# MadNLP/MadNLP.jl

Measured on AMD Instinct MI355X. Metric: IP iterations/sec + ms per factorize!/solve!, condensed KKT n≈1e4, higher is better.
Workload: dtype f64; 1 GPU; BASELINE config C3: case1354pegase-shaped sparse-condensed KKT, one instance; N=11192, m=16646, nnz(K)=68688; step = compress_J+compress_H+build_kkt+factorize (n_f=1) + inertia fetch + 2 solve_linear_system per instance; algorithm=BUNCHKAUFMAN (device: static-pivot LDL^T), outer_block=0, batch_per_gpu=1, batch_api=n/a (one instance), parallelism=1 GPU(s) x 1 independent instance(s)

## Files before the change

### madnlp.jl_amd/_lib.py

```python
from __future__ import annotations

import ctypes as C
import os
import subprocess

_HERE = os.path.dirname(os.path.abspath(__file__))
CSRC = os.path.join(_HERE, "csrc")
LIBDIR = os.path.join(_HERE, "lib")
LIBPATH = os.path.join(LIBDIR, "libmadnlp_hip.so")
_LIB_OVERRIDE = os.environ.get("MNK_LIBPATH")
SOURCES = ["gemm_f64.hip", "dag.hip", "dag_plan.hip", "dag_batch.hip", "factor.hip", "factor_plan.hip", "solve.hip", "ls.hip", "ls_alt.hip", "sparse_kkt.hip", "dense_kkt.hip", "bk.hip", "schur.hip", "ipm_vec.hip", "opf_eval.hip", "qr.hip", "lu.hip", "evd.hip", "qn.hip", "tape_eval.hip", "nlp_scale.hip"]
HEADERS = ["common.h", "ls.h", "dag_plan.h", "factor_plan.h", "kkt_vec.h", "gemm_tile.h", "leaf64.h", "ipm_handle.h", os.path.join("..", "..", "include", "madnlp_hip.h")]

MNK_HOST, MNK_DEVICE = 0, 1
MNK_BUNCHKAUFMAN, MNK_LU, MNK_QR, MNK_CHOLESKY, MNK_LDL, MNK_EVD = 1, 2, 3, 4, 5, 6
MNK_SC_JT, MNK_SC_HESS, MNK_SC_AUG, MNK_SC_DIAGBUF = 0, 1, 2, 3
MNK_QN_BFGS, MNK_QN_DAMPED_BFGS = 1, 2


def _stale() -> bool:
    if not os.path.exists(LIBPATH):
        return True
    t = os.path.getmtime(LIBPATH)
    deps = [os.path.join(CSRC, s) for s in SOURCES + HEADERS]
    return any(os.path.exists(d) and os.path.getmtime(d) > t for d in deps)


FILE_FLAGS = {"gemm_f64.hip": ["-mllvm", "-amdgpu-mfma-vgpr-form"], "dag.hip": ["-mllvm", "-amdgpu-mfma-vgpr-form"],
              "bk.hip": ["-mllvm", "-amdgpu-mfma-vgpr-form"]}


def build(force: bool = False, verbose: bool = False) -> str:
    if not force and not _stale():
        return LIBPATH
    from concurrent.futures import ThreadPoolExecutor
    hipcc = os.environ.get("HIPCC", "/opt/rocm/bin/hipcc")
    os.makedirs(LIBDIR, exist_ok=True)
    objdir = os.path.join(LIBDIR, "obj")
    os.makedirs(objdir, exist_ok=True)
    base = [hipcc, "--offload-arch=gfx950", "-O3", "-std=c++17", "-fPIC"]

    def compile_one(src):
        obj = os.path.join(objdir, src.replace(".hip", ".o"))
        cmd = base + FILE_FLAGS.get(src, []) + ["-c", os.path.join(CSRC, src), "-o", obj]
        if verbose:
# ... 240 lines not shown
```

### madnlp.jl_amd/csrc/ls.h

```cpp
#pragma once
#include <algorithm>
#include <functional>
#include <memory>
#include <string>
#include <vector>

#include "common.h"
#include "dag_plan.h"
#include "factor_plan.h"

struct mnk_sc {
    mnk_ctx* ctx = nullptr;
    int64_t n = 0, m = 0, nnzj = 0, nnzh = 0;
    int64_t nnz_jt = 0, nnz_hess = 0, nnz_aug = 0, len_jptr = 0;
    std::vector<int32_t> jt_colptr, jt_rowval, h_colptr, h_rowval, aug_colptr, aug_rowval;
    std::vector<int32_t> tile_env;
    mnk::DevBuf<int32_t> d_tile_env;
    std::vector<int32_t> tile_envh;
    mnk::DevBuf<int32_t> d_tile_envh;
    std::vector<int64_t> jt_map, h_map;
    std::vector<int32_t> d_dst, d_src, hp_dst, hp_src, j_dst, j_c, j_k, j_l;
    mnk::DevBuf<int32_t> jt_seg_ptr, jt_seg_src, h_seg_ptr, h_seg_src;
    mnk::DevBuf<int32_t> aug_hptr, aug_hsrc;
    mnk::DevBuf<int32_t> aug_dsrc;
// ... 167 lines not shown
    double bk_growth_tol = 64.0, bk_growth_tol_qd = 1e8;
    double last_growth = 0.0;
    int64_t last_sign_changes = 0;
    int count = 0;
    mnk::DevBuf<unsigned long long> amax_dev;
    bool wanted(const mnk_ls* ls) const;
    unsigned long long* growth_word(const mnk_ls* ls) const;
    bool guard_fetched(const mnk_ls* ls) const;
    bool may_take_over(const mnk_ls* ls) const;
    void note_growth(double am, double dm, int64_t sign_changes) { last_growth = am > 0.0 ? dm / am : (dm > 0.0 ? HUGE_VAL : 0.0); last_sign_changes = sign_changes; }
    bool grew() const { return !(last_growth <= (last_sign_changes <= 1 ? bk_growth_tol_qd : bk_growth_tol)); }
    int run(mnk_ls* ls);
    int permute(mnk_ls* ls, double* x, double* tmp, bool forward);
    int dsolve(mnk_ls* ls, double* y);
    int inertia(mnk_ls* ls, unsigned long long* out_dev);
    int read_pivots(mnk_ls* ls, int32_t* perm_host, double* doff_host);
    bool multi_last() const { return ran_multi; }
    int mw_fallbacks() const { return n_mw_fallbacks; }
   private:
    int factor(mnk_ls* ls, bool multi);
    mnk::DevBuf<int> perm, ptype;
    mnk::DevBuf<double> doff, dcoup, work;
    mnk::DevBuf<char> state;
    mnk::DevBuf<double> wv, tmp; mnk::DevBuf<unsigned long long> msg; mnk::DevBuf<int> aux;
    bool ran_multi = false, mw_blocked = false;
    int n_mw_fallbacks = 0;
};

struct SolveState {
    int persistent_solve = 1;
    int solve512 = 0;
    int linv_mfma = 1;
    long ps_spin_limit = 6000000;
    int debug_ps_missing = -1;
    mnk::DevBuf<double> linv512, linv512t, linv512tmp;
    mnk::DevBuf<unsigned long long> trace;
    int create();
    void destroy();
    int* abort_word() const { return abort; }
    bool abort_raised() const { return abort && *abort != 0; }
    bool take_abort();
    int poll_buffer() const { return pub_next; }
    bool reset_due(int b) { const bool due = !pub_clean[b]; pub_clean[b] = true; return due; }
    void dirtied(int b) { pub_clean[b] = false; }
    void solve_queued(bool other_cleared) { pub_clean[pub_next] = false; pub_clean[pub_next ^ 1] = other_cleared; pub_next ^= 1; }
   private:
    int* abort = nullptr;
    int pub_next = 0;
    bool pub_clean[2] = {false, false};
};

struct mnk_ls {
    mnk_ctx* ctx = nullptr;
    int64_t N = 0, Np = 0, ld = 0, ldw = 0, nbo = 512;
    bool nbo_auto = true;
    int algo = MNK_LDL;
    double pivot_tol = 0.0;
    int lookahead = 1;
    int share = 1;
    int small_tiles = 400;
    int64_t single_rows = 2560;
    mnk::DevBuf<int> tile_ctr;
    mnk::DevBuf<double> fact, wbuf[2], linv, dblk, inv16, linv256, linv256t, dvec, dinv, xwork;
    SpareFill spare;
    int epoch = 0;
    mnk::DevBuf<int> flag_p;
// ... 124 lines not shown
```

### madnlp.jl_amd/csrc/ls.hip

```cpp
#include <cstdarg>
#include <cstdlib>
#include <atomic>
#include <map>
#include <mutex>

#include <cfloat>
#include "ls.h"

namespace mnk {

static thread_local std::string g_err;
void set_error(const char* fmt, ...) {
    char buf[1024];
    va_list ap;
    va_start(ap, fmt);
    vsnprintf(buf, sizeof(buf), fmt, ap);
    va_end(ap);
    g_err = buf;
}

__global__ __launch_bounds__(256) void fill_lower_kernel(double* __restrict__ F, int64_t ld, int64_t N, int64_t Np) {
    const int64_t col = blockIdx.x;
    const int64_t first = (col / PAD) * PAD;
    const int64_t r = first + ((int64_t)blockIdx.y * 256 + threadIdx.x) * 2;
// ... 669 lines not shown
    if (!strcmp(key, "accept_only_pd")) { ls->accept_only_pd = value != 0; return 0; }
    if (!strcmp(key, "probe")) { ls->probe.on = value != 0; return 0; }
    if (!strcmp(key, "early_reject")) { ls->early_reject = value != 0; return 0; }
    if (!strcmp(key, "dag_debug")) {
        ls->dag_debug = value != 0.0;
        if (ls->dag_debug && !ls->dag_dbg.p) {
            if (ls->dag_dbg.alloc(8 * 128 + 16 * 1024)) return -2;
            MNK_HIP(hipMemset(ls->dag_dbg.p, 0, (8 * 128 + 16 * 1024) * sizeof(int)));
        }
        return 0;
    }
    if (!strcmp(key, "bk_max_wgs")) {
        MNK_REQUIRE(value >= 0.0 && value <= 256.0, "bk_max_wgs must be in 0..256");
        ls->bk.bk_max_wgs = (int)value;
        return 0;
    }
    if (!strcmp(key, "bk_spin_limit")) {
        MNK_REQUIRE(value >= 1024.0, "bk_spin_limit must be at least 1024");
        ls->bk.bk_spin_limit = (long)value;
        return 0;
    }
    if (!strcmp(key, "debug_bk_missing")) { ls->bk.debug_bk_missing = (int)value; return 0; }
    if (!strcmp(key, "bk_growth_tol")) {
        MNK_REQUIRE(value > 1.0, "bk_growth_tol must be > 1");
        ls->bk.bk_growth_tol = value;
        return 0;
    }
    if (!strcmp(key, "bk_growth_tol_qd")) {
        MNK_REQUIRE(value > 1.0, "bk_growth_tol_qd must be > 1");
        ls->bk.bk_growth_tol_qd = value;
        return 0;
    }
    if (!strcmp(key, "persistent_solve")) { ls->solves.persistent_solve = value != 0.0; return 0; }
    if (!strcmp(key, "ps_spin_limit")) {
        MNK_REQUIRE(value >= 1024.0, "ps_spin_limit must be at least 1024");
        ls->solves.ps_spin_limit = (long)value;
        return 0;
    }
    if (!strcmp(key, "debug_pp_missing")) { ls->debug_pp_missing = (int)value; return 0; }
    if (!strcmp(key, "debug_ps_missing")) { ls->solves.debug_ps_missing = (int)value; return 0; }
    if (!strcmp(key, "solve_trace")) {
        if (value != 0.0) {
            int rc = ls->solves.trace.alloc((size_t)(ls->Np / 64) * 8);
            if (rc) return rc;
            MNK_HIP(hipMemset(ls->solves.trace.p, 0, (size_t)(ls->Np / 64) * 8 * sizeof(unsigned long long)));
        } else {
            ls->solves.trace.release();
        }
        return 0;
    }
    set_error("mnk_ls_set_option: unknown option '%s'", key);
    return -1;
}

static int ensure_wbuf(mnk_ls* ls) {
    if (ls->algo != MNK_LDL || ls->wbuf[0].p) return 0;
    const size_t cnt = (size_t)ls->ldw * std::min<int64_t>(mnk_ls_effective_nbo(ls), ls->Np) + SLACK;
    int rc = ls->wbuf[0].alloc(cnt);
    if (!rc && mnk_ls_effective_nbo(ls) < ls->Np) rc = ls->wbuf[1].alloc(cnt);
    return rc;
}

static unsigned long long* amax_word(mnk_ls* ls) {
    if (!ls->bk.wanted(ls)) return nullptr;
    if (!ls->bk.amax_dev.p && ls->bk.amax_dev.alloc(AMAX_WORDS)) return nullptr;
    (void)hipMemsetAsync(ls->bk.amax_dev.p, 0, AMAX_WORDS * sizeof(unsigned long long), ls->ctx->stream);
// ... 108 lines not shown
}

static int probe_leading_block(mnk_ls* ls, mnk_sc* sc, bool* rejected) {
    *rejected = false;
    if (!(ls->probe.on && ls->early_reject && ls->accept_only_pd && ls->algo == MNK_LDL && ls->N == sc->n && !mnk_batch_active())) return 0;
    const int64_t m = ls->probe.order_due(ls->N);
    mnk_ls* c = m > 0 ? ls->probe.child(ls, m) : nullptr;
    if (c == nullptr) return 0;
    int rc = mnk_ls_factorize_sc_async(c, sc);
    if (!rc) rc = mnk_ls_fetch_info(c);
    if (rc) return rc;
    const FactorVerdict& cv = c->verdict;
    if (cv.npos == m && cv.nzero == 0 && cv.nneg == 0) { ++ls->probe.misses; return 0; }
    ++ls->probe.hits;
    ls->verdict.reject_early(cv.npos, cv.nzero, ls->N, cv.usable() ? m - 1 : cv.early_reject_col);
    ls->probe.note_verdict(true, ls->verdict.early_reject_col, ls->N);
    *rejected = true;
    return 0;
}

mnk_ls* LeadingBlockProbe::child(mnk_ls* ls, int64_t m) {
    if (ls_child == nullptr || order != m) {
        destroy();
        if (mnk_ls_create(ls->ctx, m, ls->algo, &ls_child) != 0) { (void)hipGetLastError(); ls_child = nullptr; return nullptr; }
        ls_child->probe.on = 0;
        ls_child->accept_only_pd = 1;
        ls_child->early_reject = 1;
        order = m;
    }
    mnk_ls* c = ls_child;
    c->pivot_tol = ls->pivot_tol;
    c->envelope = ls->envelope;
    c->envelope_half = ls->envelope_half;
    if (c->dag_xcd_queues != ls->dag_xcd_queues || c->dag_gang != ls->dag_gang) {
        c->dag_xcd_queues = ls->dag_xcd_queues;
        c->dag_gang = ls->dag_gang;
        c->plan.invalidate();
    }
    return c;
}

int mnk_ls_factorize_sc_async(mnk_ls* ls, mnk_sc* sc) {
    MNK_REQUIRE(ls && sc && sc->ctx, "mnk_ls_factorize_sc: NULL argument or host-only handle");
    MNK_REQUIRE(sc->n >= ls->N, "mnk_ls_factorize_sc: the solver's order exceeds the KKT system's");
    MNK_HIP(hipSetDevice(ls->ctx->device));
    { int rc_d = mnk_ls_sync_deferred(ls); if (rc_d) return rc_d; }
    int rc = ensure_wbuf(ls);
    if (rc) return rc;
    bool probe_rejected = false;
    rc = probe_leading_block(ls, sc, &probe_rejected);
    if (rc) return rc;
    if (!probe_rejected) {
        rc = transfer_sc(ls, sc);
        if (rc) return rc;
    }
    ls->src.persistent = true;
    ls->src.retransfer = handle_retransfer(sc->alive, [ls, sc]() { return transfer_sc(ls, sc); });
    if (probe_rejected) return 0;
    return mnk_ls_run_factorization(ls);
}

static int transfer_dense(mnk_ls* ls, const double* Adev, int64_t lda) {
    ls->src.env_dev = nullptr;
    dim3 grid((unsigned)ls->Np, (unsigned)((ls->Np + 1023) / 1024));
    hipLaunchKernelGGL(copy_lower_kernel, grid, dim3(256), 0, ls->ctx->stream, ls->fact.p, ls->ld, Adev, lda,
                       ls->N, ls->Np, amax_word(ls));
// ... 301 lines not shown
    MNK_REQUIRE(ls && L, "mnk_ls_get_factor: NULL argument");
    { int rc_d = mnk_ls_sync_deferred(ls); if (rc_d) return rc_d; }
    MNK_REQUIRE(ls->verdict.has_factorization(), "mnk_ls_get_factor: factorize first");
    { int rc_f = ensure_complete_factor(ls, "mnk_ls_get_factor"); if (rc_f) return rc_f; }
    MNK_HIP(hipSetDevice(ls->ctx->device));
    hipStream_t s = ls->ctx->stream;
    if (loc == MNK_DEVICE) {
        MNK_HIP(hipMemcpy2DAsync(L, ls->N * sizeof(double), ls->fact.p, ls->ld * sizeof(double), ls->N * sizeof(double), ls->N,
                                 hipMemcpyDeviceToDevice, s));
        if (D) MNK_HIP(hipMemcpyAsync(D, ls->dvec.p, ls->N * sizeof(double), hipMemcpyDeviceToDevice, s));
        MNK_HIP(mnk::stream_wait(s));
    } else {
        MNK_HIP(mnk::d2h_copy_2d(L, ls->N * sizeof(double), ls->fact.p, ls->ld * sizeof(double), ls->N * sizeof(double), ls->N, s));
        if (D) MNK_HIP(mnk::d2h_copy(D, ls->dvec.p, ls->N * sizeof(double), s));
    }
    return 0;
}

int mnk_ls_get_stat(mnk_ls* ls, const char* key, double* value) {
    MNK_REQUIRE(ls && key && value, "mnk_ls_get_stat: NULL argument");
    MNK_HIP(hipSetDevice(ls->ctx->device));
    { int rc_d = mnk_ls_sync_deferred(ls); if (rc_d) return rc_d; }
    if (ls->verdict.has_factorization()) {
        int rc = mnk_ls_fetch_info(ls);
        if (rc) return rc;
    }
    if (!strncmp(key, "pinned:", 7)) {
        *value = std::find(ls->env_keys.begin(), ls->env_keys.end(), std::string(key + 7)) != ls->env_keys.end() ? 1.0 : 0.0;
        return 0;
    }
    if (!strcmp(key, "panel_algo")) { *value = ls->algo_now; return 0; }
    if (!strcmp(key, "pp_fallbacks")) { *value = ls->pp.fallbacks; return 0; }
    if (!strcmp(key, "timeout_site")) { *value = ls->pp.last_site; return 0; }
    if (!strcmp(key, "probe_hits")) { *value = (double)ls->probe.hits; return 0; }
    if (!strcmp(key, "probe_misses")) { *value = (double)ls->probe.misses; return 0; }
    if (!strcmp(key, "early_rejects")) { *value = (double)ls->verdict.early_rejects; return 0; }
    if (!strcmp(key, "early_reject_redone")) { *value = (double)ls->verdict.early_reject_redone; return 0; }
    if (!strcmp(key, "early_reject_col")) { *value = (double)ls->verdict.early_reject_col; return 0; }
    if (!strcmp(key, "stall_ms_total")) { *value = ls->stall_ms_total; return 0; }
    if (!strcmp(key, "stall_ms_process")) { *value = mnk_process_stall_ms(); return 0; }
    if (!strcmp(key, "growth")) { *value = ls->bk.last_growth; return 0; }
    if (!strcmp(key, "sign_changes")) { *value = (double)ls->bk.last_sign_changes; return 0; }
    if (!strcmp(key, "bk_count")) { *value = ls->bk.count; return 0; }
    if (!strcmp(key, "evd_sweeps")) { *value = ls->alt ? ls->alt->stat(key) : 0.0; return 0; }
    if (!strcmp(key, "bk_panel_multi")) { *value = ls->bk.multi_last() ? 1.0 : 0.0; return 0; }
    if (!strcmp(key, "bk_mw_fallbacks")) { *value = ls->bk.mw_fallbacks(); return 0; }
    if (!strcmp(key, "dag_bulk_wgs")) { *value = ls->ctx->dag_cus > 0 ? mnk_ctx_bulk_wgs(ls->ctx, ls->ctx->dag_cus, 3) : 0; return 0; }
    if (!strcmp(key, "dag_ntasks")) { *value = ls->plan.list.size(); return 0; }
    if (!strcmp(key, "dag_ntasks1")) { *value = ls->plan.list.n1; return 0; }
    if (!strcmp(key, "dag_js2")) { *value = ls->plan.key.js2; return 0; }
    if (!strcmp(key, "dag_nq")) { *value = std::max(ls->plan.nq[0], ls->plan.nq[1]); return 0; }
    if (!strcmp(key, "dag_steals")) {
        int st[2] = {0, 0};
        if (ls->plan.qheads.p != nullptr)
            for (int ph = 0; ph < 2; ++ph)
                MNK_HIP(mnk::d2h_copy(&st[ph], ls->plan.qheads.p + ph * mnk::DAG_QHEAD_WORDS + mnk::DAG_NQ * mnk::DAG_QHEAD_STRIDE, sizeof(int), ls->ctx->stream));
        *value = (double)st[0] + (double)st[1];
        return 0;
    }
    if (!strcmp(key, "env_ksteps") || !strcmp(key, "env_ksteps_skipped")) {
        int gate = 1;
        if (ls->env_used && ls->env_word.p) MNK_HIP(mnk::d2h_copy(&gate, ls->env_word.p + 1, sizeof(int), ls->ctx->stream));
        int64_t cnt[2] = {0, 0};
        mnk::dag_env_count(ls->plan.list, ls->env_used && gate == 0 ? ls->src.env_host.data() : nullptr, (int)ls->src.env_host.size(), cnt);
        *value = (double)(!strcmp(key, "env_ksteps") ? cnt[0] : cnt[1]);
        return 0;
// ... 37 lines not shown
```

### madnlp.jl_amd/csrc/solve.hip

```cpp
#include <mutex>

#include <atomic>

#include "gemm_tile.h"
#include "ls.h"

namespace mnk {

constexpr int SB = 256;
typedef double v2d __attribute__((ext_vector_type(2)));

__device__ __forceinline__ void mm64x16_acc(const double* As, const double* Bs, double (&c)[4], int ty, int tx) {
#pragma unroll 8
    for (int k = 0; k < 64; ++k) {
        const double b = Bs[tx * 64 + k];
#pragma unroll
        for (int i = 0; i < 4; ++i) c[i] = fma(As[k * 64 + 4 * ty + i], b, c[i]);
    }
}

template <int S>
__global__ __launch_bounds__(256) void linv_tri_kernel(const double* __restrict__ F, int64_t ld,
                                                      const double* __restrict__ Linv64, double* __restrict__ Inv,
                                                      double* __restrict__ InvT, int64_t Np,
                                                      const int* __restrict__ info, int blk0) {
    __shared__ double As[64 * 64];
    __shared__ double Bs[16 * 64];
    if (*info != 0) return;
    const int64_t blk = (int64_t)blockIdx.x + blk0;
    const int q = blockIdx.y;
    const int cs = blockIdx.z;
    const int64_t j0 = blk * S;
    const int nb = (int)((Np - j0 < S ? Np - j0 : S) / 64);
    double* out = Inv + blk * (int64_t)(S * S);
    double* outT = InvT + blk * (int64_t)(S * S);
    const int t = threadIdx.x, ty = t & 15, tx = t >> 4;
    const int col = 64 * q + 16 * cs + tx;
    for (int e = t; e < 64 * q * 16; e += 256) {
// ... 258 lines not shown
        dst[t] = __longlong_as_double((long long)u);
    }
    if (s_bad != nullptr) {
        if (bad) *s_bad = 1;
        ps_barrier();
        return *s_bad == 0;
    }
    return __syncthreads_or(bad) == 0;
}

__global__ void pad_copy_kernel(double* __restrict__ dst, const double* __restrict__ src, int64_t N, int64_t Np) {
    const int64_t k = blockIdx.x * (int64_t)blockDim.x + threadIdx.x;
    if (k < Np) dst[k] = k < N ? src[k] : 0.0;
}

__global__ void ps_reset_kernel(unsigned long long* pub, int64_t n) {
    const int64_t i = blockIdx.x * (int64_t)blockDim.x + threadIdx.x;
    if (i < n) pub[i] = ~0ull;
}

constexpr int PS_NT = 1024;
constexpr int PS_NQ = PS_NT / 64;
constexpr int PS_CW = 256 / PS_NQ;

template <bool LDL>
__device__ __forceinline__ void persistent_solve_body(
    const double* __restrict__ F, int64_t ld, const double* __restrict__ Inv, const double* __restrict__ InvT,
    const double* __restrict__ dinv, const double* xin ,
    double* xout , int64_t N,
    double* __restrict__ pub ,
    double* __restrict__ pub_other ,
    int64_t Np, int* abort_flag,
    const int* __restrict__ info, unsigned long long* __restrict__ trace ,
    int near_steps, int nap, long spin_limit, int missing_wg, const int G, const int g) {
#define PS_STAMP(blk, slot) do { if (trace != nullptr && t == 0) trace[(int64_t)(blk) * 8 + (slot)] = wall_clock64(); } while (0)
    __shared__ double run[PS_MAXOWN][64];
    __shared__ double ysol[PS_MAXOWN][64];
    __shared__ double xs[256];
    __shared__ double part[PS_NQ][64];
    __shared__ int s_bad;
    const int t = threadIdx.x, r = t & 63, q = t >> 6;
    const int nb = (int)(Np / 64);
    const int nsteps = (nb + 3) / 4;
    const int nown = g < nb ? (nb - g + G - 1) / G : 0;
    if (pub_other != nullptr)
        for (int e = t; e < nown * 256; e += PS_NT) {
            const int m = e >> 8, arr = (e >> 6) & 3;
            reinterpret_cast<unsigned long long*>(pub_other)[(int64_t)arr * Np + (int64_t)(g + m * G) * 64 + (e & 63)] = ~0ull;
        }
    if (*info != 0) return;
    if (nown == 0) return;
    if (g == missing_wg) return;
    double* bfin = pub;
    double* ypub = pub + Np;
    double* zfin = pub + 2 * Np;
    double* xpub = pub + 3 * Np;
    for (int e = t; e < nown * 64; e += PS_NT) {
        const int64_t row = (int64_t)(g + (e >> 6) * G) * 64 + (e & 63);
        run[e >> 6][e & 63] = row < N ? xin[row] : 0.0;
    }
    if (t == 0) s_bad = 0;
    __syncthreads();

    double a[PS_CW];
    double d[PS_CW];
    auto dot_chunk = [&](const double (&v)[PS_CW], bool active) {
        double s0 = 0.0, s1 = 0.0, s2 = 0.0, s3 = 0.0;
        if (active) {
            const double* xq = xs + q * PS_CW;
#pragma unroll
            for (int j = 0; j < PS_CW; j += 4) {
                s0 = fma(v[j], xq[j], s0);
                s1 = fma(v[j + 1], xq[j + 1], s1);
                s2 = fma(v[j + 2], xq[j + 2], s2);
                s3 = fma(v[j + 3], xq[j + 3], s3);
            }
        }
        part[q][r] = (s0 + s1) + (s2 + s3);
    };
    auto reduce_parts = [&](int c) {
        double sm = 0.0;
#pragma unroll
        for (int u = 0; u < PS_NQ; ++u) sm += part[u][c];
        return sm;
    };
    const int qb = (q * PS_CW) >> 6;

    int m0 = 0;
    bool have_d = false;
    bool pub_b = false;
    for (int k = 0; k < nsteps && m0 < nown; ++k) {
        const int b0 = 4 * k, nbk = nb - b0 < 4 ? nb - b0 : 4;
        int i = g + m0 * G;
        if (i < b0 + nbk) {
            const int li = i - b0;
            if (!have_d) {
                const double* Mk = Inv + (int64_t)k * (SB * SB) + (li * 64 + r) + (int64_t)(q * PS_CW) * SB;
                if (qb <= li) {
#pragma unroll
                    for (int j = 0; j < PS_CW; ++j) d[j] = Mk[(int64_t)j * SB];
                }
            }
            if (!pub_b && t < 64) ps_publish(bfin + (int64_t)i * 64 + t, run[m0][t]);
            if (t < 64) xs[li * 64 + t] = run[m0][t];
            if (!ps_gather(bfin + (int64_t)b0 * 64, li * 64, xs, abort_flag, spin_limit, false, 6, &s_bad)) return;
            PS_STAMP(i, 3);
            dot_chunk(d, qb <= li);
            ps_barrier();
            if (t < 64) {
                const double v = reduce_parts(t);
                ps_publish(ypub + (int64_t)i * 64 + t, v);
                ysol[m0][t] = v;
            }
            PS_STAMP(i, 4);
            have_d = false;
            pub_b = false;
            ++m0;
            if (m0 >= nown) break;
            i = g + m0 * G;
        }
        const bool diag_next = i < b0 + nbk + 4;
        {
            const double* Fs = F + ((int64_t)i * 64 + r) + ((int64_t)b0 * 64 + q * PS_CW) * ld;
            if (qb < nbk) {
#pragma unroll
                for (int j = 0; j < PS_CW; ++j) a[j] = Fs[(int64_t)j * ld];
            }
            if (!have_d && i < b0 + nbk + 4 * PS_DAHEAD) {
                const int li = i & 3;
                const double* Mk = Inv + (int64_t)(i >> 2) * (SB * SB) + (li * 64 + r) + (int64_t)(q * PS_CW) * SB;
                if (qb <= li) {
#pragma unroll
                    for (int j = 0; j < PS_CW; ++j) d[j] = Mk[(int64_t)j * SB];
                }
                have_d = true;
            }
        }
        if (diag_next) PS_STAMP(i, 0);
        if (!ps_gather(ypub + (int64_t)b0 * 64, nbk * 64, xs, abort_flag, spin_limit, i >= b0 + nbk + 4 * near_steps, nap, &s_bad)) return;
        if (diag_next) PS_STAMP(i, 1);
        for (int m = m0; m < nown; ++m) {
            const int im = g + m * G;
            if (m > m0 && qb < nbk) {
                const double* Fs = F + ((int64_t)im * 64 + r) + ((int64_t)b0 * 64 + q * PS_CW) * ld;
#pragma unroll
                for (int j = 0; j < PS_CW; ++j) a[j] = Fs[(int64_t)j * ld];
            }
            dot_chunk(a, qb < nbk);
            ps_barrier();
            if (t < 64) {
                const double v = run[m][t] - reduce_parts(t);
                run[m][t] = v;
                if (m == m0 && diag_next) ps_publish(bfin + (int64_t)im * 64 + t, v);
            }
            if (m == m0 && diag_next) PS_STAMP(im, 2);
            if (m + 1 < nown) ps_barrier();
        }
        pub_b = diag_next;
    }

    __syncthreads();
    for (int e = t; e < nown * 64; e += PS_NT) {
        const int m = e >> 6, c = e & 63;
        const double y = ysol[m][c];
        run[m][c] = LDL ? y * dinv[(int64_t)(g + m * G) * 64 + c] : y;
    }
    __syncthreads();
    const int lane = t & 63, sub = lane & 15, colq = lane >> 4, rc = q & 3, cg = q >> 2;
    int m1 = nown - 1;
    have_d = false;
    pub_b = false;
    for (int k = nsteps - 1; k >= 0 && m1 >= 0; --k) {
        const int b0 = 4 * k, nbk = nb - b0 < 4 ? nb - b0 : 4;
        int i = g + m1 * G;
        if (i >= b0) {
            const int li = i - b0;
            const bool act = qb >= li && qb < nbk;
            if (!have_d) {
                const double* Mk = InvT + (int64_t)k * (SB * SB) + (li * 64 + r) + (int64_t)(q * PS_CW) * SB;
                if (act) {
#pragma unroll
                    for (int j = 0; j < PS_CW; ++j) d[j] = Mk[(int64_t)j * SB];
                }
            }
            if (!pub_b && t < 64) ps_publish(zfin + (int64_t)i * 64 + t, run[m1][t]);
            if (t < 64) xs[li * 64 + t] = run[m1][t];
            if (!ps_gather(zfin + (int64_t)(i + 1) * 64, (nbk - 1 - li) * 64, xs + (li + 1) * 64, abort_flag, spin_limit, false, 6, &s_bad)) return;
            dot_chunk(d, act);
            ps_barrier();
            if (t < 64) {
                const double v = reduce_parts(t);
                ps_publish(xpub + (int64_t)i * 64 + t, v);
                if ((int64_t)i * 64 + t < N) xout[(int64_t)i * 64 + t] = v;
            }
            have_d = false;
            pub_b = false;
            --m1;
            if (m1 < 0) break;
            i = g + m1 * G;
        }
        auto load_slice = [&](int im, double (&dst)[PS_CW], int bs) {
            const double* Fs = F + ((int64_t)bs * 64 + 64 * rc + 4 * sub) + ((int64_t)im * 64 + cg * 16 + colq) * ld;
#pragma unroll
            for (int p = 0; p < 4; ++p) {
                const v2d lo = *reinterpret_cast<const v2d*>(Fs + (int64_t)(4 * p) * ld);
                const v2d hi = *reinterpret_cast<const v2d*>(Fs + (int64_t)(4 * p) * ld + 2);
                dst[4 * p] = lo[0];
                dst[4 * p + 1] = lo[1];
                dst[4 * p + 2] = hi[0];
                dst[4 * p + 3] = hi[1];
            }
        };
        const bool diag_next = i >= b0 - 4;
        if (rc < nbk) load_slice(i, a, b0);
        if (!have_d && i >= b0 - 4 * PS_DAHEAD) {
            const int li = i & 3;
            const double* Mk = InvT + (int64_t)(i >> 2) * (SB * SB) + (li * 64 + r) + (int64_t)(q * PS_CW) * SB;
            if (qb >= li) {
#pragma unroll
                for (int j = 0; j < PS_CW; ++j) d[j] = Mk[(int64_t)j * SB];
            }
            have_d = true;
        }
        if (!ps_gather(xpub + (int64_t)b0 * 64, nbk * 64, xs, abort_flag, spin_limit, i < b0 - 4 * near_steps, nap, &s_bad)) return;
        for (int m = m1; m >= 0; --m) {
            const int im = g + m * G;
            if (m < m1 && rc < nbk) load_slice(im, a, b0);
            if (rc < nbk) {
                const double x0 = xs[64 * rc + 4 * sub], x1 = xs[64 * rc + 4 * sub + 1],
                             x2 = xs[64 * rc + 4 * sub + 2], x3 = xs[64 * rc + 4 * sub + 3];
#pragma unroll
                for (int p = 0; p < 4; ++p) {
                    double sp = (a[4 * p] * x0 + a[4 * p + 1] * x1) + (a[4 * p + 2] * x2 + a[4 * p + 3] * x3);
                    sp += __shfl_xor(sp, 1);
                    sp += __shfl_xor(sp, 2);
                    if ((sub & 3) == 0) part[rc * 4 + (sub >> 2)][cg * 16 + 4 * p + colq] = sp;
                }
            } else if (lane < 16) {
#pragma unroll
                for (int u = 0; u < 4; ++u) part[rc * 4 + u][cg * 16 + lane] = 0.0;
            }
            ps_barrier();
            if (t < 64) {
                const double v = run[m][t] - reduce_parts(t);
                run[m][t] = v;
                if (m == m1 && diag_next) ps_publish(zfin + (int64_t)im * 64 + t, v);
            }
            if (m > 0) ps_barrier();
        }
        pub_b = diag_next;
    }
#undef PS_STAMP
}

template <bool LDL>
__global__ __launch_bounds__(PS_NT) void persistent_solve_kernel(
    const double* __restrict__ F, int64_t ld, const double* __restrict__ Inv, const double* __restrict__ InvT,
    const double* __restrict__ dinv, const double* xin, double* xout, int64_t N, double* __restrict__ pub,
    double* __restrict__ pub_other, int64_t Np, int* abort_flag, const int* __restrict__ info,
    unsigned long long* __restrict__ trace, int near_steps, int nap, long spin_limit, int missing_wg) {
    persistent_solve_body<LDL>(F, ld, Inv, InvT, dinv, xin, xout, N, pub, pub_other, Np, abort_flag, info, trace, near_steps, nap,
                               spin_limit, missing_wg, (int)gridDim.x, (int)blockIdx.x);
}

struct PsSys {
    const double* F;
    int64_t ld;
    const double* Inv;
    const double* InvT;
    const double* dinv;
    const double* xin;
    double* xout;
    int64_t N;
    double* pub;
    double* pub_other;
    int* abort_flag;
    const int* info;
};
typedef const PsSys __attribute__((address_space(4))) * PsSysP;

template <bool LDL>
__global__ __launch_bounds__(PS_NT) void persistent_solve_multi_kernel(const PsSys* __restrict__ sys, int G, int64_t Np, int near_steps,
                                                                      int nap, long spin_limit) {
    const int isys = (int)blockIdx.x / G, g = (int)blockIdx.x % G;
    const PsSysP y = (PsSysP)(uintptr_t)(sys + isys);
    persistent_solve_body<LDL>(y->F, y->ld, y->Inv, y->InvT, y->dinv, y->xin, y->xout, y->N, y->pub, y->pub_other, Np, y->abort_flag,
                               y->info, nullptr, near_steps, nap, spin_limit, -1, G, g);
}

__global__ void ps_set_sys_kernel(PsSys rec, PsSys* __restrict__ dst) { *dst = rec; }


constexpr int P5_RB = 32, P5_NBS = 16, P5_STEP = 512, P5_NQ = 32, P5_CW = 16;

template <bool LDL>
__global__ __launch_bounds__(PS_NT) void persistent_solve512_kernel(
    const double* __restrict__ F, int64_t ld, const double* __restrict__ Inv, const double* __restrict__ InvT,
    const double* __restrict__ dinv, double* __restrict__ xio, double* __restrict__ pub, int64_t Np, int* abort_flag,
    const int* __restrict__ info, int near_steps, int nap, long spin_limit, int missing_wg) {
    __shared__ double run[PS_MAXOWN][P5_RB];
    __shared__ double ysol[PS_MAXOWN][P5_RB];
    __shared__ double xs[P5_STEP];
    __shared__ double part[P5_NQ][P5_RB];
    if (*info != 0) return;
    const int t = threadIdx.x, r = t & 31, q = t >> 5;
    const int G = gridDim.x, g = blockIdx.x;
    const int nb = (int)(Np / P5_RB);
    const int nsteps = (nb + P5_NBS - 1) / P5_NBS;
    const int nown = g < nb ? (nb - g + G - 1) / G : 0;
    if (nown == 0) return;
    if (g == missing_wg) return;
    double* bfin = pub;
    double* ypub = pub + Np;
    double* zfin = pub + 2 * Np;
    double* xpub = pub + 3 * Np;
    for (int e = t; e < nown * P5_RB; e += PS_NT) run[e >> 5][e & 31] = xio[(int64_t)(g + (e >> 5) * G) * P5_RB + (e & 31)];
    __syncthreads();

    double a[P5_CW], d[P5_CW];
    auto dot_chunk = [&](const double (&v)[P5_CW], bool active) {
// ... 292 lines not shown
    return true;
}

int mnk_ls_run_solve(mnk_ls* ls, double* xdev, double* xuser) {
    hipStream_t s = ls->ctx->stream;
    const int64_t Np = ls->Np, ld = ls->ld, N = ls->N;
    const int ldl = ls->algo == MNK_LDL;
    const int64_t nb64 = Np / 64;
    const int G = (int)std::min<int64_t>(nb64, ls->ctx->num_cu);
    const bool bk = ls->verdict.is_pivoted();
    const bool persistent = !bk && ls->solves.persistent_solve && G >= 1 && (nb64 + G - 1) / G <= PS_MAXOWN && (G >= 4 || nb64 <= G);
    const int64_t nb32 = Np / P5_RB;
    const int G5 = (int)std::min<int64_t>(nb32, ls->ctx->num_cu);
    const bool use512 = persistent && ls->solves.solve512 && ls->solves.linv512.p && (nb32 + G5 - 1) / G5 <= PS_MAXOWN && (G5 >= P5_NBS || nb32 <= G5);
    const bool direct = persistent && !use512;
    auto stage_in = [&]() -> int {
        if (xuser != nullptr) hipLaunchKernelGGL(pad_copy_kernel, dim3((unsigned)((Np + 255) / 256)), dim3(256), 0, s, xdev, xuser, N, Np);
        MNK_HIP(hipGetLastError());
        return 0;
    };
    auto stage_out = [&]() -> int {
        if (xuser != nullptr) MNK_HIP(hipMemcpyAsync(xuser, xdev, N * sizeof(double), hipMemcpyDeviceToDevice, s));
        return 0;
    };
    if (!direct) {
        int rc = stage_in();
        if (rc) return rc;
    }
    if (bk) {
        ls->solves.dirtied(0);
        int rc = ls->bk.permute(ls, xdev, xdev + 2 * Np, true);
        if (rc) return rc;
    }
    if (persistent) {
        int rc = mnk_persist_begin(ls->ctx, s);
        if (rc) return rc;
        const int ps_near = PS_NEAR, ps_nap = 6;
        double* pubs[2] = {xdev + 2 * Np, xdev + 6 * Np};
        auto ensure_clean = [&](int b) {
            if (ls->solves.reset_due(b))
                hipLaunchKernelGGL(ps_reset_kernel, dim3((unsigned)((4 * Np + 255) / 256)), dim3(256), 0, s,
                                   reinterpret_cast<unsigned long long*>(pubs[b]), 4 * Np);
        };
        if (use512) {
            ls->solves.dirtied(0);
            ensure_clean(0);
            double* pub = pubs[0];
            if (ldl)
                hipLaunchKernelGGL(persistent_solve512_kernel<true>, dim3(G5), dim3(PS_NT), 0, s, ls->fact.p, ld, ls->solves.linv512.p,
                                   ls->solves.linv512t.p, ls->dinv.p, xdev, pub, Np, ls->solves.abort_word(), ls->info_dev.p, ps_near, ps_nap,
                                   ls->solves.ps_spin_limit, ls->solves.debug_ps_missing);
            else
                hipLaunchKernelGGL(persistent_solve512_kernel<false>, dim3(G5), dim3(PS_NT), 0, s, ls->fact.p, ld, ls->solves.linv512.p,
                                   ls->solves.linv512t.p, ls->dinv.p, xdev, pub, Np, ls->solves.abort_word(), ls->info_dev.p, ps_near, ps_nap,
                                   ls->solves.ps_spin_limit, ls->solves.debug_ps_missing);
            ls->solves.dirtied(0);
            rc = hipGetLastError() == hipSuccess ? 0 : -2;
            rc = mnk_persist_end(ls->ctx, s, rc);
            return rc ? rc : stage_out();
        }
        const int cur = ls->solves.poll_buffer(), oth = cur ^ 1;
        ensure_clean(cur);
        const double* xin = xuser != nullptr ? xuser : xdev;
        double* xout = xuser != nullptr ? xuser : xdev;
        const int64_t nio = xuser != nullptr ? N : Np;
        if (ldl)
            hipLaunchKernelGGL(persistent_solve_kernel<true>, dim3(G), dim3(PS_NT), 0, s, ls->fact.p, ld, ls->linv256.p,
                               ls->linv256t.p, ls->dinv.p, xin, xout, nio, pubs[cur], pubs[oth], Np, ls->solves.abort_word(), ls->info_dev.p,
                               ls->solves.trace.p, ps_near, ps_nap, ls->solves.ps_spin_limit, ls->solves.debug_ps_missing);
        else
            hipLaunchKernelGGL(persistent_solve_kernel<false>, dim3(G), dim3(PS_NT), 0, s, ls->fact.p, ld,
                               ls->linv256.p, ls->linv256t.p, ls->dinv.p, xin, xout, nio, pubs[cur], pubs[oth], Np, ls->solves.abort_word(),
                               ls->info_dev.p, ls->solves.trace.p, ps_near, ps_nap, ls->solves.ps_spin_limit,
                               ls->solves.debug_ps_missing);
        ls->solves.solve_queued(ls->solves.debug_ps_missing < 0);
        rc = hipGetLastError() == hipSuccess ? 0 : -2;
        return mnk_persist_end(ls->ctx, s, rc);
    }
    double* b = xdev;
    double* y = xdev + Np;
    const int64_t nsteps = (Np + SB - 1) / SB;
    for (int64_t k = 0; k < nsteps; ++k) {
        const int64_t j0 = k * SB;
        const int ncol = (int)std::min<int64_t>(SB, Np - j0);
        hipLaunchKernelGGL(diag256_kernel, dim3(1), dim3(1024), 0, s, ls->linv256.p + k * (int64_t)(SB * SB), b + j0,
                           y + j0, 0, ncol);
        const int64_t below = Np - j0 - ncol;
        if (below > 0)
            hipLaunchKernelGGL(fwd_panel_kernel, dim3((unsigned)((below + 63) / 64)), dim3(256), 0, s, ls->fact.p, ld,
                               y, b, j0, ncol, Np);
    }
    if (bk) {
        int rc = ls->bk.dsolve(ls, y);
        if (rc) return rc;
    } else if (ldl)
        hipLaunchKernelGGL(scale_vec_kernel, dim3((unsigned)((Np + 255) / 256)), dim3(256), 0, s, y, ls->dinv.p, Np);
    for (int64_t k = nsteps - 1; k >= 0; --k) {
        const int64_t j0 = k * SB;
        const int nrow = (int)std::min<int64_t>(SB, Np - j0);
        hipLaunchKernelGGL(diag256_kernel, dim3(1), dim3(1024), 0, s, ls->linv256t.p + k * (int64_t)(SB * SB), y + j0,
                           b + j0, 1, nrow);
        if (j0 > 0)
            hipLaunchKernelGGL(bwd_panel_kernel, dim3((unsigned)(j0 / 64)), dim3(256), 0, s, ls->fact.p, ld, b, y, j0,
                               nrow);
    }
    MNK_HIP(hipGetLastError());
    if (bk) {
        ls->solves.dirtied(0);
// ... 22 lines not shown

bool mnk_solve_defer(mnk_ls* ls, double* xuser) {
    if (!t_sbatch.active || !solve_eligible(ls)) return false;
    if (!ls->ev_defer && hipEventCreateWithFlags(&ls->ev_defer, hipEventDisableTiming) != hipSuccess) { (void)hipGetLastError(); return false; }
    if (hipEventRecord(ls->ev_defer, ls->ctx->stream) != hipSuccess) { (void)hipGetLastError(); return false; }
    t_sbatch.pend.push_back({ls, xuser});
    return true;
}

static int solve_batch_launch(const std::vector<SolveReq>& v) {
    const int q = (int)v.size();
    mnk_ls* l0 = v[0].ls;
    mnk_ctx* c0 = l0->ctx;
    hipStream_t h = c0->stream;
    MNK_HIP(hipSetDevice(c0->device));
    const int64_t Np = l0->Np, nb64 = Np / 64;
    const int G = (int)std::min<int64_t>(nb64, c0->num_cu / q);
    SolveBatchBuffers& B = g_sbatch[c0->device & 63];
    for (const SolveReq& r : v)
        if (r.ls->ctx->stream != h) MNK_HIP(hipStreamWaitEvent(h, r.ls->ev_defer, 0));
    int rc = mnk_persist_begin(c0, h);
    if (rc) return rc;
    auto body = [&]() -> int {
        if (B.sys.n < sizeof(PsSys) * PS_BATCH_MAXQ && B.sys.alloc(sizeof(PsSys) * PS_BATCH_MAXQ)) return -2;
        if (!B.ev) MNK_HIP(hipEventCreateWithFlags(&B.ev, hipEventDisableTiming));
        PsSys* dsys = reinterpret_cast<PsSys*>(B.sys.p);
        for (int i = 0; i < q; ++i) {
            mnk_ls* ls = v[i].ls;
            double* pubs[2] = {ls->xwork.p + 2 * Np, ls->xwork.p + 6 * Np};
            const int cur = ls->solves.poll_buffer(), oth = cur ^ 1;
            if (ls->solves.reset_due(cur))
                hipLaunchKernelGGL(ps_reset_kernel, dim3((unsigned)((4 * Np + 255) / 256)), dim3(256), 0, h,
                                   reinterpret_cast<unsigned long long*>(pubs[cur]), 4 * Np);
            PsSys rec{ls->fact.p, ls->ld, ls->linv256.p, ls->linv256t.p, ls->dinv.p, v[i].x, v[i].x, ls->N, pubs[cur], pubs[oth],
                      ls->solves.abort_word(), ls->info_dev.p};
            hipLaunchKernelGGL(ps_set_sys_kernel, dim3(1), dim3(1), 0, h, rec, dsys + i);
            ls->solves.solve_queued(true);
        }
        const bool ldl = l0->algo == MNK_LDL;
        if (ldl)
            hipLaunchKernelGGL(persistent_solve_multi_kernel<true>, dim3((unsigned)(q * G)), dim3(PS_NT), 0, h, dsys, G, Np, PS_NEAR, 6, l0->solves.ps_spin_limit);
        else
            hipLaunchKernelGGL(persistent_solve_multi_kernel<false>, dim3((unsigned)(q * G)), dim3(PS_NT), 0, h, dsys, G, Np, PS_NEAR, 6, l0->solves.ps_spin_limit);
        MNK_HIP(hipGetLastError());
        return 0;
    };
    rc = body();
    rc = mnk_persist_end(c0, h, rc);
    if (rc) return rc;
    bool other = false;
    for (const SolveReq& r : v) other = other || r.ls->ctx->stream != h;
    if (other) {
        MNK_HIP(hipEventRecord(B.ev, h));
        for (const SolveReq& r : v)
            if (r.ls->ctx->stream != h) MNK_HIP(hipStreamWaitEvent(r.ls->ctx->stream, B.ev, 0));
    }
    return 0;
}

static int solve_batch_flush() {
    std::vector<SolveReq> pend;
    pend.swap(t_sbatch.pend);
    int rc_all = 0;
    while (!pend.empty()) {
        mnk_ls* l0 = pend.front().ls;
        const int64_t nb64 = l0->Np / 64;
        const int g4 = (int)std::max<int64_t>(1, std::min<int64_t>(nb64, l0->ctx->num_cu / 4));
        const int maxq = std::max(1, std::min(PS_BATCH_MAXQ, l0->ctx->num_cu / g4));
        std::vector<SolveReq> g, rest;
        for (const SolveReq& r : pend) {
// ... 40 lines not shown
```

Before: 110.2 it/s.

## Prefetch next factor slice into LDS during persistent-solve gather spin

```diff
diff --git a/madnlp.jl_amd/_lib.py b/madnlp.jl_amd/_lib.py
--- a/madnlp.jl_amd/_lib.py
+++ b/madnlp.jl_amd/_lib.py
@@ -10,7 +10,7 @@
 LIBPATH = os.path.join(LIBDIR, "libmadnlp_hip.so")
 _LIB_OVERRIDE = os.environ.get("MNK_LIBPATH")
 SOURCES = ["gemm_f64.hip", "dag.hip", "dag_plan.hip", "dag_batch.hip", "factor.hip", "factor_plan.hip", "solve.hip", "ls.hip", "ls_alt.hip", "sparse_kkt.hip", "dense_kkt.hip", "bk.hip", "schur.hip", "ipm_vec.hip", "opf_eval.hip", "qr.hip", "lu.hip", "evd.hip", "qn.hip", "tape_eval.hip", "nlp_scale.hip"]
-HEADERS = ["common.h", "ls.h", "dag_plan.h", "factor_plan.h", "kkt_vec.h", "gemm_tile.h", "leaf64.h", "ipm_handle.h", os.path.join("..", "..", "include", "madnlp_hip.h")]
+HEADERS = ["common.h", "ls.h", "dag_plan.h", "factor_plan.h", "kkt_vec.h", "gemm_tile.h", "leaf64.h", "ipm_handle.h", "solve_stage.h", os.path.join("..", "..", "include", "madnlp_hip.h")]
 
 MNK_HOST, MNK_DEVICE = 0, 1
 MNK_BUNCHKAUFMAN, MNK_LU, MNK_QR, MNK_CHOLESKY, MNK_LDL, MNK_EVD = 1, 2, 3, 4, 5, 6
diff --git a/madnlp.jl_amd/csrc/ls.h b/madnlp.jl_amd/csrc/ls.h
--- a/madnlp.jl_amd/csrc/ls.h
+++ b/madnlp.jl_amd/csrc/ls.h
@@ -223,6 +223,8 @@
     int solve512 = 0;
     int linv_mfma = 1;
     long ps_spin_limit = 6000000;
+    int solve_stage = 1;
+    long persistent_solves = 0, staged_solves = 0;
     int debug_ps_missing = -1;
     mnk::DevBuf<double> linv512, linv512t, linv512tmp;
     mnk::DevBuf<unsigned long long> trace;
diff --git a/madnlp.jl_amd/csrc/ls.hip b/madnlp.jl_amd/csrc/ls.hip
--- a/madnlp.jl_amd/csrc/ls.hip
+++ b/madnlp.jl_amd/csrc/ls.hip
@@ -725,6 +725,11 @@
         return 0;
     }
     if (!strcmp(key, "persistent_solve")) { ls->solves.persistent_solve = value != 0.0; return 0; }
+    if (!strcmp(key, "solve_stage")) {
+        MNK_REQUIRE(value == 0.0 || value == 1.0 || value == 2.0, "solve_stage must be 0, 1 or 2");
+        ls->solves.solve_stage = (int)value;
+        return 0;
+    }
     if (!strcmp(key, "ps_spin_limit")) {
         MNK_REQUIRE(value >= 1024.0, "ps_spin_limit must be at least 1024");
         ls->solves.ps_spin_limit = (long)value;
@@ -899,6 +904,7 @@
     c->pivot_tol = ls->pivot_tol;
     c->envelope = ls->envelope;
     c->envelope_half = ls->envelope_half;
+    c->solves.solve_stage = ls->solves.solve_stage;
     if (c->dag_xcd_queues != ls->dag_xcd_queues || c->dag_gang != ls->dag_gang) {
         c->dag_xcd_queues = ls->dag_xcd_queues;
         c->dag_gang = ls->dag_gang;
@@ -1266,6 +1272,9 @@
     if (!strcmp(key, "panel_algo")) { *value = ls->algo_now; return 0; }
     if (!strcmp(key, "pp_fallbacks")) { *value = ls->pp.fallbacks; return 0; }
     if (!strcmp(key, "timeout_site")) { *value = ls->pp.last_site; return 0; }
+    if (!strcmp(key, "solve_stage")) { *value = ls->solves.solve_stage; return 0; }
+    if (!strcmp(key, "persistent_solves")) { *value = (double)ls->solves.persistent_solves; return 0; }
+    if (!strcmp(key, "staged_solves")) { *value = (double)ls->solves.staged_solves; return 0; }
     if (!strcmp(key, "probe_hits")) { *value = (double)ls->probe.hits; return 0; }
     if (!strcmp(key, "probe_misses")) { *value = (double)ls->probe.misses; return 0; }
     if (!strcmp(key, "early_rejects")) { *value = (double)ls->verdict.early_rejects; return 0; }
diff --git a/madnlp.jl_amd/csrc/solve.hip b/madnlp.jl_amd/csrc/solve.hip
--- a/madnlp.jl_amd/csrc/solve.hip
+++ b/madnlp.jl_amd/csrc/solve.hip
@@ -4,6 +4,7 @@
 
 #include "gemm_tile.h"
 #include "ls.h"
+#include "solve_stage.h"
 
 namespace mnk {
 
@@ -328,13 +329,15 @@
     double* __restrict__ pub_other ,
     int64_t Np, int* abort_flag,
     const int* __restrict__ info, unsigned long long* __restrict__ trace ,
-    int near_steps, int nap, long spin_limit, int missing_wg, const int G, const int g) {
+    int near_steps, int nap, long spin_limit, int missing_wg, const int G, const int g,
+    const int stage ) {
 #define PS_STAMP(blk, slot) do { if (trace != nullptr && t == 0) trace[(int64_t)(blk) * 8 + (slot)] = wall_clock64(); } while (0)
     __shared__ double run[PS_MAXOWN][64];
     __shared__ double ysol[PS_MAXOWN][64];
     __shared__ double xs[256];
     __shared__ double part[PS_NQ][64];
     __shared__ int s_bad;
+    __shared__ __attribute__((aligned(16))) double stage_buf[stage::BYTES / 8];
     const int t = threadIdx.x, r = t & 63, q = t >> 6;
     const int nb = (int)(Np / 64);
     const int nsteps = (nb + 3) / 4;
@@ -381,10 +384,43 @@
         return sm;
     };
     const int qb = (q * PS_CW) >> 6;
+    const unsigned stage_lds = (unsigned)(uintptr_t)(__attribute__((address_space(3))) char*)reinterpret_cast<char*>(stage_buf);
+    auto stage_request = [&](const double* src, int lds_bytes) {
+        const unsigned to = __builtin_amdgcn_readfirstlane(stage_lds + (unsigned)lds_bytes);
+        unsigned keep;
+        asm volatile("s_mov_b32 %0, m0\n\ts_mov_b32 m0, %2\n\ts_nop 0\n\tglobal_load_lds_dwordx4 %1, off\n\ts_mov_b32 m0, %0"
+                     : "=&s"(keep)
+                     : "v"(src), "s"(to)
+                     : "memory");
+    };
+    auto stage_fwd = [&](int i, int bs, int nbs) {
+        if (qb < nbs) {
+            asm volatile("s_waitcnt lgkmcnt(0)" ::: "memory");
+            const stage::Elem e = stage::fwd_req_elem(q, 0, r);
+            const double* Fs = F + ((int64_t)i * 64 + e.row) + ((int64_t)bs * 64 + e.col) * ld;
+#pragma unroll
+            for (int n = 0; n < stage::REQS; ++n) stage_request(Fs + (int64_t)(2 * n) * ld, stage::fwd_req_base(q, n));
+        }
+    };
+    auto unstage_fwd = [&](int nbs) {
+        asm volatile("s_waitcnt vmcnt(0)" ::: "memory");
+        if (qb < nbs) {
+            const unsigned at = stage_lds + (unsigned)stage::fwd_read_bytes(r, q, 0);
+#pragma unroll
+            for (int j = 0; j < PS_CW; ++j)
+                asm volatile("ds_read_b64 %0, %1 offset:%2" : "=v"(a[j]) : "v"(at), "n"(stage::fwd_read_bytes(0, 0, j)));
+            asm volatile("s_waitcnt lgkmcnt(0)"
+                         : "+v"(a[0]), "+v"(a[1]), "+v"(a[2]), "+v"(a[3]), "+v"(a[4]), "+v"(a[5]), "+v"(a[6]), "+v"(a[7]), "+v"(a[8]),
+                           "+v"(a[9]), "+v"(a[10]), "+v"(a[11]), "+v"(a[12]), "+v"(a[13]), "+v"(a[14]), "+v"(a[15])
+                         :
+                         : "memory");
+        }
+    };
 
     int m0 = 0;
     bool have_d = false;
     bool pub_b = false;
+    bool staged = false;
     for (int k = 0; k < nsteps && m0 < nown; ++k) {
         const int b0 = 4 * k, nbk = nb - b0 < 4 ? nb - b0 : 4;
         int i = g + m0 * G;
@@ -418,7 +454,7 @@
         const bool diag_next = i < b0 + nbk + 4;
         {
             const double* Fs = F + ((int64_t)i * 64 + r) + ((int64_t)b0 * 64 + q * PS_CW) * ld;
-            if (qb < nbk) {
+            if (!staged && qb < nbk) {
 #pragma unroll
                 for (int j = 0; j < PS_CW; ++j) a[j] = Fs[(int64_t)j * ld];
             }
@@ -432,9 +468,13 @@
                 have_d = true;
             }
         }
+        const bool stage_next = stage != 0 && !diag_next;
+        const int nbk1 = nb - b0 - 4 < 4 ? nb - b0 - 4 : 4;
+        if (stage_next && stage != 2) stage_fwd(i, b0 + 4, nbk1);
         if (diag_next) PS_STAMP(i, 0);
         if (!ps_gather(ypub + (int64_t)b0 * 64, nbk * 64, xs, abort_flag, spin_limit, i >= b0 + nbk + 4 * near_steps, nap, &s_bad)) return;
         if (diag_next) PS_STAMP(i, 1);
+        if (stage_next && stage == 2) stage_fwd(i, b0 + 4, nbk1);
         for (int m = m0; m < nown; ++m) {
             const int im = g + m * G;
             if (m > m0 && qb < nbk) {
@@ -453,6 +493,8 @@
             if (m + 1 < nown) ps_barrier();
         }
         pub_b = diag_next;
+        if (stage_next) unstage_fwd(nbk1);
+        staged = stage_next;
     }
 
     __syncthreads();
@@ -466,6 +508,7 @@
     int m1 = nown - 1;
     have_d = false;
     pub_b = false;
+    staged = false;
     for (int k = nsteps - 1; k >= 0 && m1 >= 0; --k) {
         const int b0 = 4 * k, nbk = nb - b0 < 4 ? nb - b0 : 4;
         int i = g + m1 * G;
@@ -507,8 +550,25 @@
                 dst[4 * p + 3] = hi[1];
             }
         };
+        auto stage_bwd = [&](int im, int bs) {
+            asm volatile("s_waitcnt lgkmcnt(0)" ::: "memory");
+            const stage::Elem e = stage::bwd_req_elem(q, 0, lane);
+            const double* Fs = F + ((int64_t)bs * 64 + e.row) + ((int64_t)im * 64 + e.col) * ld;
+#pragma unroll
+            for (int n = 0; n < stage::REQS; ++n) stage_request(Fs + (int64_t)(4 * (n >> 1)) * ld + 2 * (n & 1), stage::bwd_req_base(q, n));
+        };
+        auto unstage_bwd = [&]() {
+            asm volatile("s_waitcnt vmcnt(0)" ::: "memory");
+#pragma unroll
+            for (int n = 0; n < stage::REQS; ++n) {
+                const v2d v = *reinterpret_cast<const v2d*>(reinterpret_cast<const char*>(stage_buf) + stage::bwd_read_bytes(q, lane, n));
+                a[2 * n] = v[0];
+                a[2 * n + 1] = v[1];
+            }
+        };
         const bool diag_next = i >= b0 - 4;
-        if (rc < nbk) load_slice(i, a, b0);
+        const bool stage_next = stage != 0 && !diag_next;
+        if (!staged && rc < nbk) load_slice(i, a, b0);
         if (!have_d && i >= b0 - 4 * PS_DAHEAD) {
             const int li = i & 3;
             const double* Mk = InvT + (int64_t)(i >> 2) * (SB * SB) + (li * 64 + r) + (int64_t)(q * PS_CW) * SB;
@@ -518,7 +578,9 @@
             }
             have_d = true;
         }
+        if (stage_next && stage != 2) stage_bwd(i, b0 - 4);
         if (!ps_gather(xpub + (int64_t)b0 * 64, nbk * 64, xs, abort_flag, spin_limit, i < b0 - 4 * near_steps, nap, &s_bad)) return;
+        if (stage_next && stage == 2) stage_bwd(i, b0 - 4);
         for (int m = m1; m >= 0; --m) {
             const int im = g + m * G;
             if (m < m1 && rc < nbk) load_slice(im, a, b0);
@@ -545,6 +607,8 @@
             if (m > 0) ps_barrier();
         }
         pub_b = diag_next;
+        if (stage_next) unstage_bwd();
+        staged = stage_next;
     }
 #undef PS_STAMP
 }
@@ -554,9 +618,9 @@
     const double* __restrict__ F, int64_t ld, const double* __restrict__ Inv, const double* __restrict__ InvT,
     const double* __restrict__ dinv, const double* xin, double* xout, int64_t N, double* __restrict__ pub,
     double* __restrict__ pub_other, int64_t Np, int* abort_flag, const int* __restrict__ info,
-    unsigned long long* __restrict__ trace, int near_steps, int nap, long spin_limit, int missing_wg) {
+    unsigned long long* __restrict__ trace, int near_steps, int nap, long spin_limit, int missing_wg, int stage) {
     persistent_solve_body<LDL>(F, ld, Inv, InvT, dinv, xin, xout, N, pub, pub_other, Np, abort_flag, info, trace, near_steps, nap,
-                               spin_limit, missing_wg, (int)gridDim.x, (int)blockIdx.x);
+                               spin_limit, missing_wg, (int)gridDim.x, (int)blockIdx.x, stage);
 }
 
 struct PsSys {
@@ -572,6 +636,7 @@
     double* pub_other;
     int* abort_flag;
     const int* info;
+    int stage;
 };
 typedef const PsSys __attribute__((address_space(4))) * PsSysP;
 
@@ -581,7 +646,7 @@
     const int isys = (int)blockIdx.x / G, g = (int)blockIdx.x % G;
     const PsSysP y = (PsSysP)(uintptr_t)(sys + isys);
     persistent_solve_body<LDL>(y->F, y->ld, y->Inv, y->InvT, y->dinv, y->xin, y->xout, y->N, y->pub, y->pub_other, Np, y->abort_flag,
-                               y->info, nullptr, near_steps, nap, spin_limit, -1, G, g);
+                               y->info, nullptr, near_steps, nap, spin_limit, -1, G, g, y->stage);
 }
 
 __global__ void ps_set_sys_kernel(PsSys rec, PsSys* __restrict__ dst) { *dst = rec; }
@@ -940,6 +1005,8 @@
         int rc = ls->bk.permute(ls, xdev, xdev + 2 * Np, true);
         if (rc) return rc;
     }
+    const int stage = ls->solves.solve_stage;
+    MNK_REQUIRE(stage == 0 || (reinterpret_cast<uintptr_t>(ls->fact.p) % 16 == 0 && ld % 2 == 0), "solve: the factor is not 16-byte aligned");
     if (persistent) {
         int rc = mnk_persist_begin(ls->ctx, s);
         if (rc) return rc;
@@ -975,13 +1042,15 @@
         if (ldl)
             hipLaunchKernelGGL(persistent_solve_kernel<true>, dim3(G), dim3(PS_NT), 0, s, ls->fact.p, ld, ls->linv256.p,
                                ls->linv256t.p, ls->dinv.p, xin, xout, nio, pubs[cur], pubs[oth], Np, ls->solves.abort_word(), ls->info_dev.p,
-                               ls->solves.trace.p, ps_near, ps_nap, ls->solves.ps_spin_limit, ls->solves.debug_ps_missing);
+                               ls->solves.trace.p, ps_near, ps_nap, ls->solves.ps_spin_limit, ls->solves.debug_ps_missing, stage);
         else
             hipLaunchKernelGGL(persistent_solve_kernel<false>, dim3(G), dim3(PS_NT), 0, s, ls->fact.p, ld,
                                ls->linv256.p, ls->linv256t.p, ls->dinv.p, xin, xout, nio, pubs[cur], pubs[oth], Np, ls->solves.abort_word(),
                                ls->info_dev.p, ls->solves.trace.p, ps_near, ps_nap, ls->solves.ps_spin_limit,
-                               ls->solves.debug_ps_missing);
+                               ls->solves.debug_ps_missing, stage);
         ls->solves.solve_queued(ls->solves.debug_ps_missing < 0);
+        ls->solves.persistent_solves += 1;
+        ls->solves.staged_solves += stage != 0;
         rc = hipGetLastError() == hipSuccess ? 0 : -2;
         return mnk_persist_end(ls->ctx, s, rc);
     }
@@ -1070,10 +1139,14 @@
             if (ls->solves.reset_due(cur))
                 hipLaunchKernelGGL(ps_reset_kernel, dim3((unsigned)((4 * Np + 255) / 256)), dim3(256), 0, h,
                                    reinterpret_cast<unsigned long long*>(pubs[cur]), 4 * Np);
+            const int stage = ls->solves.solve_stage;
+            MNK_REQUIRE(stage == 0 || (reinterpret_cast<uintptr_t>(ls->fact.p) % 16 == 0 && ls->ld % 2 == 0), "solve: the factor is not 16-byte aligned");
             PsSys rec{ls->fact.p, ls->ld, ls->linv256.p, ls->linv256t.p, ls->dinv.p, v[i].x, v[i].x, ls->N, pubs[cur], pubs[oth],
-                      ls->solves.abort_word(), ls->info_dev.p};
+                      ls->solves.abort_word(), ls->info_dev.p, stage};
             hipLaunchKernelGGL(ps_set_sys_kernel, dim3(1), dim3(1), 0, h, rec, dsys + i);
             ls->solves.solve_queued(true);
+            ls->solves.persistent_solves += 1;
+            ls->solves.staged_solves += stage != 0;
         }
         const bool ldl = l0->algo == MNK_LDL;
         if (ldl)
diff --git a/madnlp.jl_amd/csrc/solve_stage.h b/madnlp.jl_amd/csrc/solve_stage.h
--- /dev/null
+++ b/madnlp.jl_amd/csrc/solve_stage.h
@@ -0,0 +1,33 @@
+#pragma once
+
+namespace mnk {
+namespace stage {
+
+constexpr int ROWS = 64;
+constexpr int STEP = 256;
+constexpr int WAVES = 16;
+constexpr int REQS = 8;
+constexpr int REQ_BYTES = 1024;
+constexpr int WAVE_BYTES = REQS * REQ_BYTES;
+constexpr int BYTES = WAVES * WAVE_BYTES;
+
+struct Elem { int row, col; };
+
+constexpr int lane_bytes(int lane) { return 16 * lane; }
+
+constexpr int fwd_req_base(int q, int n) { return ((16 * q + 2 * n) * ROWS) * 8; }
+constexpr Elem fwd_req_elem(int q, int n, int lane) { return Elem{2 * (lane & 31), 16 * q + 2 * n + (lane >> 5)}; }
+constexpr int fwd_read_bytes(int r, int q, int j) { return ((16 * q + j) * ROWS + r) * 8; }
+constexpr Elem fwd_read_elem(int r, int q, int j) { return Elem{r, 16 * q + j}; }
+
+constexpr int bwd_req_base(int q, int n) { return q * WAVE_BYTES + n * REQ_BYTES; }
+constexpr Elem bwd_req_elem(int q, int n, int lane) {
+    return Elem{64 * (q & 3) + 4 * (lane & 15) + 2 * (n & 1), 16 * (q >> 2) + 4 * (n >> 1) + (lane >> 4)};
+}
+constexpr int bwd_read_bytes(int q, int lane, int n) { return bwd_req_base(q, n) + lane_bytes(lane); }
+constexpr Elem bwd_read_elem(int q, int lane, int v) {
+    return Elem{64 * (q & 3) + 4 * (lane & 15) + (v & 3), 16 * (q >> 2) + 4 * (v >> 2) + (lane >> 4)};
+}
+
+}
+}
```

Result: no change. 111.2 it/s, median of 6 (+0.9%).
